# httpsLiem/Spectrogram-YOLOv11

Measured on AMD Instinct MI355X. Metric: spectrogram-images/sec (train fwd+bwd) YOLOv11-s 640², bs=64, 1/2/4/8 GPU, higher is better.
Workload: dtype f16; 1 GPU; configs[2]: YOLOv11-s train fwd+bwd (+clip, SGD-nesterov, EMA) from synthetic IQ through the HIP STFT/log-mel producer; model=yolo11s.yaml, imgsz=640, batch_per_gpu=64, global_batch=64, parallelism=dp1, weights=random-init, nc=80

## Files before the change

### include/sy11.h

```cpp
#ifndef SY11_H
#define SY11_H
#include <stddef.h>
#include <stdint.h>
#ifdef __cplusplus
extern "C" {
#endif

#define SY11_VERSION 100

enum sy11_status { SY11_OK = 0, SY11_EINVAL = -1, SY11_EUNSUPPORTED = -2, SY11_ELAUNCH = -3 };
enum sy11_dtype { SY11_F32 = 0, SY11_F16 = 1, SY11_BF16 = 2, SY11_U8 = 3  };

#define SY11_EPI_SILU 1u
#define SY11_EPI_ACCUM 2u
#define SY11_EPI_OUT_F32 4u

typedef struct sy11_conv_desc {
  int32_t dtype;
  int32_t B, IH, IW, C;
  int32_t x_ld;
  int32_t OH, OW, N;
  int32_t y_ld;
  int32_t KH, KW, SH, SW, PH, PW, DH, DW;
  int32_t groups;
// ... 24 lines not shown
  float* running_var;
  float* mean;
  float* rstd;
  float* scale;
  float* shift;
  int32_t* ticket;
  float eps, momentum;
  double count;
} sy11_bn_tail;
int sy11_conv2d_fwd_bn(const sy11_conv_desc* d, const void* x, const void* w, void* y, float* stat_sum, float* stat_sq,
                       const sy11_bn_tail* bn, void* stream);

int sy11_conv2d_dgrad(const sy11_conv_desc* d, const void* dy, int32_t dy_ld, const void* wt, void* dx, void* stream);

int sy11_conv2d_wgrad(const sy11_conv_desc* d, const void* x, const void* dy, int32_t dy_ld, float* dw, void* stream);

int sy11_weight_transpose(int32_t dtype, int32_t N, int32_t T, int32_t C, const void* w, void* wt, void* stream);

int sy11_weight_transpose_multi(int32_t dtype, int32_t nlayers, int32_t total_tiles, const void* desc, const void* src,
                                void* dst, void* stream);

int sy11_stem_conv_fwd(const sy11_conv_desc* d, const float* x_nchw, const void* w, const float* bias, void* y,
                       float* stat_sum, float* stat_sq, void* stream);
int sy11_stem_conv_fwd_bn(const sy11_conv_desc* d, const float* x_nchw, const void* w, void* y, float* stat_sum,
                          float* stat_sq, const sy11_bn_tail* bn, void* stream);
int sy11_stem_conv_wgrad(const sy11_conv_desc* d, const float* x_nchw, const void* dy, int32_t dy_ld, float* dw,
                         void* stream);


int sy11_bn_finalize(int32_t C, int32_t stat_slots, double count, const float* stat_sum, const float* stat_sq, const float* gamma,
// ... 186 lines not shown
```

### spectrogram-yolov11_amd/csrc/elementwise.hip

```cpp
#include "common.h"
#include "tune.h"
#include "det.h"
#include <type_traits>

template <int I, int N, typename F>
__device__ __forceinline__ void sy11_static_for(F&& f) {
  if constexpr (I < N) {
    f(std::integral_constant<int, I>{});
    sy11_static_for<I + 1, N>(f);
  }
}


template <typename T, int VEC> struct Vec {
  T v[VEC];
};
template <typename T, int VEC>
__device__ __forceinline__ void vload(const T* p, float* f) {
  if constexpr (VEC == 1) {
    f[0] = ElemTraits<T>::to_f(*p);
  } else {
    typedef T vt __attribute__((ext_vector_type(VEC)));
    const vt v = *(const vt*)p;
#pragma unroll
// ... 1134 lines not shown
  float* src = partials;
  int cl = clean ? 1 : 0;
  long sstride = stride;
  float* ping = scratch;
  while (rows > 256) {
    const long nr = (rows + 63) / 64;
    float* dst = ping;
    hipLaunchKernelGGL((fold_stage_kernel<false>), dim3(cdiv(N, 64), (unsigned)nr), dim3(256), 0, st, rows, N, src, sstride, dst, 64L, 0L, 0L, (float*)nullptr, cl);
    src = dst; sstride = N; rows = nr; cl = 0;
    ping = dst + nr * N;
  }
  hipLaunchKernelGGL((fold_stage_kernel<true>), dim3(cdiv(N, 64), 1), dim3(256), 0, st, rows, N, src, sstride, out, rows, 0L, 0L, (float*)nullptr, cl);
  SY11_LAUNCH_CHECK("fold_rows");
  return SY11_OK;
}
```

### spectrogram-yolov11_amd/csrc/wgrad.hip

```cpp
#include "common.h"
#include "tune.h"
#include "det.h"
#include <stdlib.h>

struct WgradArgs {
  const void* x;
  const void* dy;
  float* dw;
  int M, N, K, C, T;
  int x_ld, dy_ld;
  int IH, IW, OH, OW, sy, sx;
  int tiles_k;
  unsigned x_bytes, dy_bytes;
  unsigned mag_ow, mag_oh;
  int tiles, total;
  int pix_per_split;
  long dw_split_stride;
  signed char tap_dy[64];
  signed char tap_dx[64];
};

template <bool STORE>
__device__ __forceinline__ void dw_out(float* p, float v) {
  if (STORE) *p = v; else atomicAdd(p, v);
// ... 640 lines not shown
static int wgrad3x3p_sp(const WgradArgs& a, int ws) { return (ws >= 40 && a.OH % (160 / ws) == 0) ? 160 : 80; }

static int cu_count() {
  static int n = 0;
  if (!n) {
    int dev = 0;
    hipDeviceProp_t p;
    n = (hipGetDevice(&dev) == hipSuccess && hipGetDeviceProperties(&p, dev) == hipSuccess && p.multiProcessorCount > 0) ? p.multiProcessorCount : 256;
  }
  return n;
}

constexpr int WGRAD_NCFG = SY11_WGRAD_NCFG;
static_assert(WGRAD_NCFG == 20, "configuration table and its size (tune.h) out of step");
constexpr int WGRAD_WIDE_LDS = 2 * 64 * ((128 * 2 + 64) + (256 * 2 + 64));
static int wgrad_launch_cfg(WgradArgs a, int dtype, hipStream_t st, int cfg) {
  const int kind = cfg >> 2;
  const bool psplit = kind == 2;
  const bool patch = kind == 3;
  const bool wide = kind == 4;
  if (wide && dtype == SY11_F32) SY11_FAIL(SY11_EUNSUPPORTED, "conv2d_wgrad: configuration %d is 16-bit only", cfg);
  const int patch_ws = patch ? wgrad3x3p_ws(a) : 0;
  if (patch && (!patch_ws || dtype == SY11_F32)) SY11_FAIL(SY11_EUNSUPPORTED, "conv2d_wgrad: configuration %d does not take this shape", cfg);
  const int patch_sp = patch ? wgrad3x3p_sp(a, patch_ws) : 0;
  const int tile = kind == 1 ? 128 : 64;
  const int slots = cu_count() * (wide ? 1 : patch ? (patch_sp == 80 ? 4 : 2) : (tile == 128 ? 2 : 3));
  const int target_wg = (slots << (cfg & 3)) >> 2;
  const int pcb = a.C > 32 ? 64 : 32, pnb = a.N > 32 ? 64 : 32;
  a.tiles_k = patch ? cdiv(a.C, pcb) : cdiv(a.K, wide ? 256 : tile);
  const int tiles = patch ? a.tiles_k * cdiv(a.N, pnb) * 3 : a.tiles_k * cdiv(a.N, wide ? 128 : tile);
  int splits = target_wg / tiles;
  const int stage_px = patch ? patch_sp : 64;
  const int max_splits = cdiv(a.M, 8 * stage_px);
  if (splits > max_splits) splits = max_splits;
  if (splits < 1) splits = 1;
  a.pix_per_split = cdiv(cdiv(a.M, splits), stage_px) * stage_px;
  splits = cdiv(a.M, a.pix_per_split);
  a.tiles = tiles; a.total = tiles * splits;
  DetPartials dp;
  float* const dw_out = a.dw;
  const bool det = sy11_det(8) && splits > 1;
  if (det) {
    if (!dp.acquire(st, 1, splits, a.N * a.K, false)) SY11_FAIL(SY11_ELAUNCH, "conv2d_wgrad: ordered-reduction workspace unavailable (%d x %d floats)", splits, a.N * a.K);
    a.dw = dp.buf(0);
    a.dw_split_stride = (long)a.N * a.K;
  }
  a.mag_ow = (unsigned)(((1u << 20) + a.OW - 1) / a.OW);
  a.mag_oh = (unsigned)(((1u << 20) + a.OH - 1) / a.OH);
  dim3 grid(cdiv(a.total, 8) * 8), block(256);
  if (wide) {
    static bool attr_set = false;
    if (!attr_set) {
      if (hipFuncSetAttribute((const void*)wgrad16w_kernel<_Float16>, hipFuncAttributeMaxDynamicSharedMemorySize, WGRAD_WIDE_LDS) != hipSuccess ||
          hipFuncSetAttribute((const void*)wgrad16w_kernel<__bf16>, hipFuncAttributeMaxDynamicSharedMemorySize, WGRAD_WIDE_LDS) != hipSuccess)
        SY11_FAIL(SY11_ELAUNCH, "conv2d_wgrad: cannot raise the LDS limit to %d bytes", WGRAD_WIDE_LDS);
      attr_set = true;
// ... 21 lines not shown
    } while (0)
    if (dtype == SY11_F16) SY11_WG3(_Float16); else SY11_WG3(__bf16);
#undef SY11_WG3
#undef SY11_WG3B
  } else if (dtype == SY11_F16) {
    if (psplit) hipLaunchKernelGGL((wgrad16_kernel<_Float16, 64, true>), grid, block, 0, st, a);
    else if (tile == 128) hipLaunchKernelGGL((wgrad16_kernel<_Float16, 128>), grid, block, 0, st, a);
    else hipLaunchKernelGGL((wgrad16_kernel<_Float16, 64>), grid, block, 0, st, a);
  } else {
    if (psplit) hipLaunchKernelGGL((wgrad16_kernel<__bf16, 64, true>), grid, block, 0, st, a);
    else if (tile == 128) hipLaunchKernelGGL((wgrad16_kernel<__bf16, 128>), grid, block, 0, st, a);
    else hipLaunchKernelGGL((wgrad16_kernel<__bf16, 64>), grid, block, 0, st, a);
  }
  SY11_LAUNCH_CHECK("conv2d_wgrad");
  if (det) return dp.fold(0, dw_out);
  return SY11_OK;
}

extern "C" int sy11_conv2d_wgrad_dw(const sy11_conv_desc* d, const void* x, const void* dy, int dy_ld, float* dw, hipStream_t st);
extern "C" int sy11_conv2d_wgrad(const sy11_conv_desc* d, const void* x, const void* dy, int32_t dy_ld, float* dw,
                                 void* stream) {
  SY11_REQUIRE(d && x && dy && dw, "conv2d_wgrad: null argument");
  SY11_REQUIRE(dtype_ok(d->dtype), "conv2d_wgrad: bad dtype");
  hipStream_t st = (hipStream_t)stream;
  if (d->groups != 1 && d->groups == d->C && d->C == d->N) return sy11_conv2d_wgrad_dw(d, x, dy, dy_ld, dw, st);
  if (d->groups != 1) {
    SY11_REQUIRE(d->groups > 1 && d->C % d->groups == 0 && d->N % d->groups == 0, "conv2d_wgrad: channels not divisible by groups=%d", d->groups);
    const int cg = d->C / d->groups, ng = d->N / d->groups, es = dtype_size(d->dtype);
    sy11_conv_desc dg = *d;
    dg.groups = 1; dg.C = cg; dg.N = ng;
    for (int g = 0; g < d->groups; ++g) {
      const int rc = sy11_conv2d_wgrad(&dg, (const char*)x + (long)g * cg * es, (const char*)dy + (long)g * ng * es, dy_ld,
                                       dw + (long)g * ng * d->KH * d->KW * cg, stream);
      if (rc) return rc;
    }
    return SY11_OK;
  }
  const int esz = dtype_size(d->dtype), epc = 16 / esz;
  SY11_REQUIRE(d->KH * d->KW <= 64 && d->KH > 0 && d->KW > 0, "conv2d_wgrad: <=64 taps");
  SY11_REQUIRE(d->C % epc == 0 && d->N % epc == 0, "conv2d_wgrad: C and N must be multiples of %d", epc);
  SY11_REQUIRE(d->x_ld % epc == 0 && dy_ld % epc == 0 && d->x_ld >= d->C && dy_ld >= d->N, "conv2d_wgrad: bad pixel strides");
  SY11_REQUIRE((((uintptr_t)x | (uintptr_t)dy) & 15) == 0 && ((uintptr_t)dw & 3) == 0, "conv2d_wgrad: misaligned pointer");
  SY11_REQUIRE((long)d->B * d->IH * d->IW < (1L << 31) && (long)d->B * d->OH * d->OW < (1L << 31), "conv2d_wgrad: pixel count overflows int32");
  WgradArgs a{};
  a.x = x; a.dy = dy; a.dw = dw;
  {
    const long xb = ((long)d->B * d->IH * d->IW - 1) * d->x_ld * esz + (long)d->C * esz;
    const long db = ((long)d->B * d->OH * d->OW - 1) * dy_ld * esz + (long)d->N * esz;
    SY11_REQUIRE(xb < (1L << 31) && db < (1L << 31), "conv2d_wgrad: operand view larger than 2 GiB");
    SY11_REQUIRE((long)(d->OW + 64) * d->OW < (1L << 20) && (long)(d->OH + 64) * d->OH < (1L << 20), "conv2d_wgrad: output map larger than 960 pixels per side");
    a.x_bytes = (unsigned)xb; a.dy_bytes = (unsigned)db;
  }
  a.T = d->KH * d->KW; a.C = d->C; a.K = a.T * a.C; a.N = d->N;
  a.M = d->B * d->OH * d->OW;
  a.x_ld = d->x_ld; a.dy_ld = dy_ld;
  a.IH = d->IH; a.IW = d->IW; a.OH = d->OH; a.OW = d->OW; a.sy = d->SH; a.sx = d->SW;
  for (int r = 0; r < d->KH; ++r)
    for (int s = 0; s < d->KW; ++s) {
      a.tap_dy[r * d->KW + s] = (signed char)(r * d->DH - d->PH);
      a.tap_dx[r * d->KW + s] = (signed char)(s * d->DW - d->PW);
    }
  int cfg = ((a.N > 64 && a.K > 64 && a.M > 30000) ? 4 : 0) + 2;
  if (d->dtype != SY11_F32 && a.M >= 200000 && wgrad3x3p_ws(a)) cfg = 14;
  const int forced = sy11_opt(OPT_WGRAD_CFG);
  const int ncfg = d->dtype == SY11_F32 ? 8 : WGRAD_NCFG;
  auto patch_ok = [&](int c) { return c < 12 || (c < 16 ? wgrad3x3p_ws(a) != 0 : (a.N > 64 && a.K > 128)); };
  if (forced >= 0 && forced < ncfg && patch_ok(forced)) return wgrad_launch_cfg(a, d->dtype, st, forced);
  {
    sy11tune::Cache& cache = sy11tune::cache(1);
    static float* scratch = nullptr;
    static size_t scratch_elems = 0;
    const int key[] = {d->dtype, a.M, a.N, a.K, a.C, a.sy, a.sx, a.IW, a.OW, a.x_ld, a.dy_ld};
    const uint64_t h = sy11tune::hash(key, (int)(sizeof(key) / sizeof(int)));
    int hit;
    if (cache.get(h, &hit)) {
      if (hit >= 0 && hit < ncfg && patch_ok(hit)) cfg = hit;
    } else if (sy11tune::enabled() && !sy11tune::capturing(st)) {
      const size_t need = (size_t)a.N * a.K;
      if (need > scratch_elems) {
        if (scratch) (void)hipFree(scratch);
        scratch = nullptr; scratch_elems = 0;
        if (hipMalloc((void**)&scratch, need * sizeof(float)) == hipSuccess) scratch_elems = need; else (void)hipGetLastError();
      }
      if (scratch) {
        WgradArgs t = a;
        t.dw = scratch;
        int cands[WGRAD_NCFG], nc = 0;
        for (int c = 0; c < ncfg; ++c)
          if (patch_ok(c)) cands[nc++] = c;
        const int best = sy11tune::pick(cands, nc, [&](int c) { return wgrad_launch_cfg(t, d->dtype, st, c); }, st, "wgrad", key,
                                        (int)(sizeof(key) / sizeof(int)));
        if (best >= 0) { cache.put(h, best); cfg = best; }
      }
    }
  }
  return wgrad_launch_cfg(a, d->dtype, st, cfg);
}
```

### spectrogram-yolov11_amd/sy11/_lib.py

```python
from __future__ import annotations

import ctypes as C
import os
from pathlib import Path

_HERE = Path(__file__).resolve().parent
LIB_PATH = Path(os.environ.get("SY11_LIB", _HERE / "libsy11.so"))

F32, F16, BF16, U8 = 0, 1, 2, 3
EPI_SILU, EPI_ACCUM, EPI_OUT_F32 = 1, 2, 4


class Sy11Error(RuntimeError):
    pass


class ConvDesc(C.Structure):
    _fields_ = [(n, C.c_int32) for n in (
        "dtype", "B", "IH", "IW", "C", "x_ld", "OH", "OW", "N", "y_ld",
        "KH", "KW", "SH", "SW", "PH", "PW", "DH", "DW", "groups")] + [("flags", C.c_uint32), ("stat_slots", C.c_int32)]


class BnTail(C.Structure):
    _fields_ = [(n, C.c_void_p) for n in ("gamma", "beta", "running_mean", "running_var", "mean", "rstd", "scale", "shift", "ticket")] \
# ... 20 lines not shown
    _fields_ = [("m0", C.c_int64), ("out_off", C.c_int64), ("M", C.c_int32), ("log2d", C.c_int32), ("dphi", C.c_uint32),
                ("reserved", C.c_int32)]


_vp, _i32, _i64, _f32, _f64, _u32 = C.c_void_p, C.c_int32, C.c_int64, C.c_float, C.c_double, C.c_uint32
_dp = C.POINTER(ConvDesc)
_bp = C.POINTER(BnTail)
_op = C.POINTER(OptDesc)

SIGNATURES = {
    "sy11_conv2d_fwd": [_dp, _vp, _vp, _vp, _vp, _vp, _vp, _vp],
    "sy11_conv2d_fwd_bn": [_dp, _vp, _vp, _vp, _vp, _vp, _bp, _vp],
    "sy11_stem_conv_fwd_bn": [_dp, _vp, _vp, _vp, _vp, _vp, _bp, _vp],
    "sy11_conv2d_dgrad": [_dp, _vp, _i32, _vp, _vp, _vp],
    "sy11_conv2d_wgrad": [_dp, _vp, _vp, _i32, _vp, _vp],
    "sy11_weight_transpose": [_i32, _i32, _i32, _i32, _vp, _vp, _vp],
    "sy11_weight_transpose_multi": [_i32, _i32, _i32, _vp, _vp, _vp, _vp],
    "sy11_stem_conv_fwd": [_dp, _vp, _vp, _vp, _vp, _vp, _vp, _vp],
    "sy11_stem_conv_wgrad": [_dp, _vp, _vp, _i32, _vp, _vp],
    "sy11_bn_finalize": [_i32, _i32, _f64, _vp, _vp, _vp, _vp, _f32, _f32, _vp, _vp, _vp, _vp, _vp, _vp, _vp],
    "sy11_bn_act_fwd": [_i32, _i64, _i32, _vp, _i32, _vp, _vp, _i32, _vp, _i32, _vp, _i32, _vp],
    "sy11_bn_act_bwd_reduce": [_i32, _i64, _i32, _vp, _i32, _vp, _i32, _vp, _vp, _vp, _vp, _i32, _vp, _vp, _i32, _vp],
    "sy11_bn_act_bwd_apply": [_i32, _i64, _i32, _vp, _i32, _vp, _i32, _vp, _vp, _vp, _vp, _vp, _i32, _vp, _vp, _i32,
                              _vp, _i32, _vp, _vp, _vp],
    "sy11_bn_act_bwd_apply_res": [_i32, _i64, _i32, _vp, _i32, _vp, _i32, _vp, _vp, _vp, _vp, _vp, _i32, _vp, _vp, _i32,
                                  _vp, _i32, _vp, _vp, _vp, _i32, _i32, _vp],
    "sy11_copy2d": [_i32, _i64, _i32, _vp, _i32, _vp, _i32, _i32, _vp],
    "sy11_upsample2x_fwd": [_i32, _i32, _i32, _i32, _i32, _vp, _i32, _vp, _i32, _vp],
    "sy11_upsample2x_bwd": [_i32, _i32, _i32, _i32, _i32, _vp, _i32, _vp, _i32, _i32, _vp],
    "sy11_box_iou": [_i32, _i32, _vp, _vp, _f32, _vp, _vp],
# ... 44 lines not shown
    "sy11_tune_import": [_vp, _i64],
    "sy11_tune_clear": [],
    "sy11_peak_mfma_f16": [_i32, _i32, _vp, _vp],
    "sy11_debug_stamps": [_vp],
    "sy11_debug_stamps_persistent": [_vp],
    "sy11_opt_workspace_floats": [_i32],
    "sy11_opt_grad_norm": [_i64, _vp, _vp, _vp, _vp, _i32, _vp],
    "sy11_opt_step": [_op, _vp, _vp, _vp, _vp, _vp, _vp, _vp, _vp, _vp, _vp, _vp, _vp, _vp],
})
OTHER = {"sy11_version": ([], C.c_int), "sy11_last_error": ([], C.c_char_p),
         "sy11_nms_workspace_bytes": ([_i32], C.c_size_t),
         "sy11_nms_batched_workspace_bytes": ([_i32, _vp], C.c_size_t),
         "sy11_scan_merge_workspace_bytes": ([_i32, _i32], C.c_size_t),
         "sy11_attention_workspace_bytes": ([_i32, _i32, _i32], C.c_size_t),
         "sy11_iq_extract_tile": ([_i32], C.c_int32),
         "sy11_tune_export": ([_vp, _i64], C.c_int64)}

_lib = None


def load():
    global _lib
    if _lib is not None:
        return _lib
    if not LIB_PATH.exists():
        raise Sy11Error(f"libsy11.so not found at {LIB_PATH}: build it with "
                        f"`make -C spectrogram-yolov11_amd/csrc` (or __graft_entry__.build()). "
                        f"There is no CPU / PyTorch fallback for the hot path.")
    import torch
    lib = C.CDLL(str(LIB_PATH))
    for name, args in SIGNATURES.items():
# ... 63 lines not shown
```

### spectrogram-yolov11_amd/sy11/engine/__init__.py

```python
from __future__ import annotations

import os

from typing import List, Optional

import torch

from .. import ops


class Act:

    __slots__ = ("_data", "root", "c0", "_grad", "_ready", "raw", "req", "_dtype")

    def __init__(self, data: Optional[torch.Tensor], root: Optional["Act"] = None, c0: int = 0,
                 raw: Optional[torch.Tensor] = None, req: bool = True, dtype=None):
        self._data = data
        self.root = root
        self.c0 = c0
        self._grad = None
        self._ready = False
        self.raw = raw
        self.req = req
        self._dtype = dtype
# ... 45 lines not shown
        r = self._root_grad()
        if not r._ready:
            r._grad.zero_()
            r._ready = True
        return r._grad if self.root is None else r._grad[..., self.c0:self.c0 + self.C]

    def set_grad(self, g: torch.Tensor):
        assert self.root is None
        self._grad = g
        self._ready = True


_SIDE_WGRAD = os.environ.get("SY11_WGRAD_STREAM", "32") != "0"
_SIDE_BATCH = max(int(os.environ.get("SY11_WGRAD_STREAM", "32") or 0), 1)
_SIDE_STREAMS = {}


def _side_stream(device):
    d = torch.device(device)
    key = d.index if d.index is not None else torch.cuda.current_device()
    if key not in _SIDE_STREAMS:
        _SIDE_STREAMS[key] = torch.cuda.Stream(device=d)
    return _SIDE_STREAMS[key]


_BRANCH_STREAMS_ON = os.environ.get("SY11_BRANCH_STREAMS", "0") != "0"
_BRANCH_STREAMS = {}


def _branch_stream(device, b):
# ... 45 lines not shown
        self.pool_off = 0
        self.pool_need = 0
        self.bn_counters: List[torch.Tensor] = []
        self.capturing = False
        self.w_views = None
        self.wt_views = None
        self.w_bank = None
        self.flat_state = None
        self.side = None
        self.side_refs: List = []
        self.use_side = _SIDE_WGRAD and device is not None and torch.device(device).type == "cuda"
        self.use_branches = _BRANCH_STREAMS_ON and device is not None and torch.device(device).type == "cuda"
        self.open_branches = set()
        self.main_stream = None
        self.tape_branches: List = []

    def on_side(self, fn, *keep):
        if not self.use_side:
            fn()
            return
        if self.side is None:
            self.side = _side_stream(self.device)
            self.side_queue = []
        self.side_queue.append(fn)
        self.side_refs.append(keep)
        if len(self.side_queue) >= _SIDE_BATCH:
            self.flush_side()

    def flush_side(self):
        if self.side is None or not self.side_queue:
# ... 106 lines not shown
                v = seg.view(p.shape)
            self.views[id(p)] = v
            self.offsets[id(p)] = off
            off += pad(n)

    def begin_backward(self, device):
        if self.flat is None or self.flat.device != device:
            self._build(device)
        fresh = any(p.grad is None or p.grad.data_ptr() != self.views[id(p)].data_ptr() for p in self.params)
        if fresh:
            if not (self.external_zero and all(p.grad is not None for p in self.params)):
                self.flat.zero_()
            for p in self.params:
                p.grad = self.views[id(p)]

    def grad_krsc(self, p: torch.nn.Parameter) -> torch.Tensor:
        return self.views[id(p)].permute(0, 2, 3, 1)

    def grad_vec(self, p: torch.nn.Parameter) -> torch.Tensor:
        return self.views[id(p)]


def engine_dtype(module) -> torch.dtype:
    if torch.is_autocast_enabled("cuda"):
        return torch.get_autocast_dtype("cuda")
    return getattr(module, "_sy11_dtype", torch.float32)


def to_act(t: torch.Tensor, dtype) -> Act:
    if not t.is_cuda:
# ... 36 lines not shown
        out = module._run(ec, acts if is_list else acts[0])
        if ec.bn_counters:
            torch._foreach_add_(ec.bn_counters, 1)
        ctx.module = module
        outs, out_list = _flatten(out)
        ctx.ec, ctx.acts, ctx.outs, ctx.n_in = ec, acts, outs, n_in
        ctx.n_t = len(tensors)
        ctx.in_req = [t.requires_grad for t in ins]
        return tuple(from_act(a) for a in outs)

    @staticmethod
    def backward(ctx, *gouts):
        ec: Ctx = ctx.ec
        if ec.grads is not None:
            ec.grads.begin_backward(ec.device)
        for a, g in zip(ctx.outs, gouts):
            if g is None or a.data.dim() != 4:
                continue
            gv = g.permute(0, 2, 3, 1)
            if gv.dtype != a.data.dtype or not gv.is_contiguous():
                gv = gv.to(a.data.dtype).contiguous()
            a.set_grad(gv)
        hook = module_post_backward.get(id(ec.grads)) if ec.grads is not None else None
        mark = ec.marks.get("bucket") if (hook is not None and getattr(hook, "staged", False)) else None
        def first_bucket():
            ec.join_side()
            hook(ec.grads, 0)
        ec.run_tape(len(ec.tape) - 1, 0, mark, first_bucket if mark is not None else None)
        ec.join_side()
        ec.tape.clear()
        ctx.module.__dict__["_sy11_pool_hint"] = ec.pool_need
        gin = []
        for a, req in zip(ctx.acts, ctx.in_req):
            if req:
                g = a.grad_read().permute(0, 3, 1, 2)
                gin.append(g.float() if g.dtype != torch.float32 else g)
            else:
                gin.append(None)
        if hook is not None:
            hook(ec.grads, 1)
        return (None, None, None, None, None, *gin, *([None] * (ctx.n_t - ctx.n_in)))


module_post_backward = {}
# ... 22 lines not shown
                ec = Ctx(True, True, dtype, dev, store, module.__dict__.get("_sy11_pool_hint", 0))
                ec.capturing = True
                ec.attach_flat(module)
                acts = [to_act(t, dtype) for t in self.static_in]
                out = module._run(ec, acts if is_list else acts[0])
                if ec.bn_counters:
                    torch._foreach_add_(ec.bn_counters, 1)
            self.ec, self.acts = ec, acts
            self.outs, _ = _flatten(out)
            self.static_out = [from_act(a) for a in self.outs]
            self.static_gout = [torch.zeros_like(a.data) for a in self.outs]
            hook = module_post_backward.get(id(store))
            mark = ec.marks.get("bucket") if (hook is not None and getattr(hook, "staged", False)) else None
            if mark is not None and not (0 < mark < len(ec.tape)):
                mark = None
            self.g_bwd = torch.cuda.CUDAGraph()
            self.g_bwd2 = None
            with torch.cuda.graph(self.g_bwd, pool=self.g_fwd.pool(), stream=side, capture_error_mode=_CAPTURE_MODE):
                for a, g in zip(self.outs, self.static_gout):
                    if a.data.dim() == 4:
                        a.set_grad(g)
                ec.run_tape(len(ec.tape) - 1, mark if mark is not None else 0)
                ec.join_side()
                if mark is None:
                    self.static_gin = [a.grad_read().permute(0, 3, 1, 2) if a.req else None for a in acts]
            if mark is not None:
                self.g_bwd2 = torch.cuda.CUDAGraph()
                with torch.cuda.graph(self.g_bwd2, pool=self.g_fwd.pool(), stream=side, capture_error_mode=_CAPTURE_MODE):
                    ec.run_tape(mark - 1, 0)
                    ec.join_side()
                    self.static_gin = [a.grad_read().permute(0, 3, 1, 2) if a.req else None for a in acts]
            ec.tape.clear()
        torch.cuda.current_stream(dev).wait_stream(side)


class _GraphedFwd:

    def __init__(self, module, xs, is_list, dtype):
        dev = xs[0].device
        self.static_in = [x.detach().clone() for x in xs]
        side = torch.cuda.Stream(device=dev)
        side.wait_stream(torch.cuda.current_stream(dev))
        with torch.cuda.stream(side):
            self.g_fwd = torch.cuda.CUDAGraph()
            with torch.cuda.graph(self.g_fwd, stream=side, capture_error_mode=_CAPTURE_MODE):
# ... 113 lines not shown
```

### spectrogram-yolov11_amd/sy11/nn/modules/conv.py

```python
from __future__ import annotations

import math

import torch
import torch.nn as nn

from ... import ops
from ...engine import Act, Ctx, run_module

import os

_BN_TAIL = os.environ.get("SY11_BN_TAIL", "0") != "0"
_BN_STAT_SLOTS = max(1, int(os.environ.get("SY11_BN_STAT_SLOTS", "32")))

__all__ = ("Conv", "DWConv", "DDWConv", "Concat", "WeightedSpatialAttention", "GCT", "Fusion", "autopad")


def autopad(k, p=None, d=1):
    if d > 1:
        k = d * (k - 1) + 1 if isinstance(k, int) else [d * (x - 1) + 1 for x in k]
    if p is None:
        p = k // 2 if isinstance(k, int) else [x // 2 for x in k]
    return p

# ... 156 lines not shown
            tail = (B * OH * OW, gamma, beta, bn.eps, mom, rm, rv, mean, rstd, scale, shift, ec.zeros(max(g, 1)))
            if stem:
                ops.stem_conv_fwd_bn(x.raw, w, y, s, p, (st[0], st[1]), tail)
            else:
                ops.conv2d_fwd_bn(x.data, w, y, k, s, p, d, g, (st[0], st[1]), tail)
        else:
            if stem:
                ops.stem_conv_fwd(x.raw, w, y, s, p, stats=(st[0], st[1]))
            else:
                ops.conv2d_fwd(x.data, w, y, k, s, p, d, g, stats=(st[0], st[1]))
            ops.bn_finalize(B * OH * OW, st[0], st[1], gamma, beta, bn.eps, mom, rm, rv, mean, rstd, scale, shift)
        if track and bn.num_batches_tracked is not None:
            ec.bn_counters.append(bn.num_batches_tracked)
        ops.bn_act_fwd(y, scale, shift, out.data, silu=silu, res=res.data if res is not None else None)
        if ec.record:
            def bw():
                gs = ec.grads
                dz = out.grad_read()
                sg = ec.zeros(2, 8 if B * OH * OW >= 8192 else 1, N)
                ops.bn_act_bwd_reduce(y, dz, mean, rstd, scale, shift, silu, sg[0], sg[1])
                dy = torch.empty_like(y)
                has_bn = id(bn.weight) in gs.views
                rg, acc = res.grad_for_write() if (res is not None and res.req) else (None, False)
                ops.bn_act_bwd_apply(y, dz, mean, rstd, scale, shift, gamma, silu, sg[0], sg[1], dy,
                                     gs.grad_vec(bn.weight) if has_bn else None, gs.grad_vec(bn.bias) if has_bn else None,
                                     res_grad=rg, res_accumulate=acc)
                if id(conv.weight) in gs.views:
                    dw = gs.grad_krsc(conv.weight)
                    if stem:
                        ec.on_side(lambda: ops.stem_conv_wgrad(x.raw, dy, dw, s, p), x.raw, dy)
                    elif padded:
                        dwp = torch.zeros(tuple(w.shape), dtype=torch.float32, device=ec.device)
                        ops.conv2d_wgrad(x.data, dy, dwp, k, s, p, d, g)
                        dw.add_(dwp[..., :C1])
                    else:
                        xd = x.data
                        ec.on_side(lambda: ops.conv2d_wgrad(xd, dy, dw, k, s, p, d, g), xd, dy)
                if padded and x_real.req:
                    gp = torch.zeros_like(x.data)
                    ops.conv2d_dgrad(dy, ops.weight_transpose(w), gp, (B, OH, OW, N), k, s, p, d, 1, accumulate=True)
                    gx, acc = x_real.grad_for_write()
                    if acc:
                        gx.add_(gp[..., :C1])
                    else:
                        gx.copy_(gp[..., :C1])
                if x.req:
                    gx, acc = x.grad_for_write()
                    if g == 1 or g != C1 or g != N:
                        if ops.dgrad_leaves_holes(k, s, p, d) and not acc:
                            gx.zero_()
                            acc = True
                        wtr = ec.transposed(conv.weight, w) if g == 1 else ops.weight_transpose(w, g)
# ... 147 lines not shown
```

### spectrogram-yolov11_amd/sy11/ops.py

```python
from __future__ import annotations

import ctypes as C

import numpy as np
import torch

from . import _lib
from ._lib import EPI_ACCUM, EPI_OUT_F32, EPI_SILU, BnTail, ConvDesc, OptDesc, call

_DT = {torch.float32: _lib.F32, torch.float16: _lib.F16, torch.bfloat16: _lib.BF16}


def dt_code(t: torch.dtype) -> int:
    try:
        return _DT[t]
    except KeyError:
        raise _lib.Sy11Error(f"unsupported dtype {t}") from None


def _stream():
    return C.c_void_p(torch.cuda.current_stream().cuda_stream)


def _p(t):
# ... 98 lines not shown

def conv2d_dgrad(dy, w_or_wt, dx, y_shape, k, s=1, p=0, d=1, groups=1, accumulate=False):
    _need_gpu(dy, w_or_wt, dx)
    dsc = _desc(dx.shape, view_ld(dx), y_shape, y_shape[-1], dy.dtype, k, s, p, d, groups, EPI_ACCUM if accumulate else 0)
    call("sy11_conv2d_dgrad", C.byref(dsc), _p(dy), view_ld(dy), _p(w_or_wt), _p(dx), _stream())
    return dx


def conv2d_wgrad(x, dy, dw_f32, k, s=1, p=0, d=1, groups=1):
    _need_gpu(x, dy, dw_f32)
    if dw_f32.dtype != torch.float32 or not dw_f32.is_contiguous():
        raise _lib.Sy11Error("conv2d_wgrad: dw must be a contiguous f32 tensor")
    dsc = _desc(x.shape, view_ld(x), dy.shape, view_ld(dy), x.dtype, k, s, p, d, groups, 0)
    call("sy11_conv2d_wgrad", C.byref(dsc), _p(x), _p(dy), view_ld(dy), _p(dw_f32), _stream())
    return dw_f32


def stem_conv_fwd(x_nchw, w_krsc, y, s=2, p=1, bias=None, stats=None, silu=False):
    _need_gpu(x_nchw, w_krsc, y)
    if x_nchw.dtype != torch.float32 or not x_nchw.is_contiguous() or x_nchw.shape[1] != 3:
        raise _lib.Sy11Error("stem_conv_fwd: x must be a contiguous NCHW f32 image with 3 channels")
    B, _, IH, IW = x_nchw.shape
    slots = stats[0].shape[0] if (stats and stats[0].dim() == 2) else 1
    dsc = _desc((B, IH, IW, 3), 3, y.shape, view_ld(y), y.dtype, 3, s, p, 1, 1, EPI_SILU if silu else 0, slots)
    call("sy11_stem_conv_fwd", C.byref(dsc), _p(x_nchw), _p(w_krsc), _p(bias), _p(y), _p(stats[0]) if stats else None,
         _p(stats[1]) if stats else None, _stream())
    return y


def stem_conv_wgrad(x_nchw, dy, dw_f32, s=2, p=1):
# ... 702 lines not shown
```

Before: 3061 spectrogram-images/s.

## Store split-K wgrad partials in an arena and fold all layers in one kernel

Split-K weight-gradient kernels used to accumulate into the f32 gradient buffer with atomicAdd from every split. Now each eligible non-grouped conv writes its per-split partials with plain stores into a per-layer block of a shared arena. After backward, one batched grad_fold kernel sums the splits into the flat gradient buffer. This replaces atomic contention with plain stores and one vectorised reduction pass. The cost is extra arena memory (up to 64 MB per layer), extra read traffic for the fold, and a tuning key that now depends on whether partials are used.

```diff
diff --git a/include/sy11.h b/include/sy11.h
--- a/include/sy11.h
+++ b/include/sy11.h
@@ -62,6 +62,12 @@
 int sy11_conv2d_dgrad(const sy11_conv_desc* d, const void* dy, int32_t dy_ld, const void* wt, void* dx, void* stream);
 
 int sy11_conv2d_wgrad(const sy11_conv_desc* d, const void* x, const void* dy, int32_t dy_ld, float* dw, void* stream);
+
+int sy11_conv2d_wgrad_split(const sy11_conv_desc* d, const void* x, const void* dy, int32_t dy_ld, float* dw, float* partial,
+                            int64_t partial_floats, int32_t* splits_out, void* stream);
+int64_t sy11_conv2d_wgrad_partial_floats(const sy11_conv_desc* d);
+int sy11_grad_fold(const int64_t* table, const int32_t* work, int32_t work_count, const uint16_t* counts, int32_t n_counts,
+                   int32_t entry_base, float* flat, const float* arena, void* stream);
 
 int sy11_weight_transpose(int32_t dtype, int32_t N, int32_t T, int32_t C, const void* w, void* wt, void* stream);
 
diff --git a/spectrogram-yolov11_amd/csrc/elementwise.hip b/spectrogram-yolov11_amd/csrc/elementwise.hip
--- a/spectrogram-yolov11_amd/csrc/elementwise.hip
+++ b/spectrogram-yolov11_amd/csrc/elementwise.hip
@@ -1172,3 +1172,61 @@
   SY11_LAUNCH_CHECK("fold_rows");
   return SY11_OK;
 }
+
+struct GradFoldCounts { uint16_t c[256]; };
+__global__ __launch_bounds__(256) void grad_fold_kernel(const int64_t* __restrict__ table, const int32_t* __restrict__ work, const GradFoldCounts cnt,
+                                                        int entry_base, float* __restrict__ flat, const float* __restrict__ arena) {
+  const int e = work[2 * blockIdx.x], chunk = work[2 * blockIdx.x + 1];
+  const int S = cnt.c[e - entry_base];
+  if (S == 0) return;
+  const int64_t* ent = table + 3L * e;
+  const long i = ((long)chunk * 256 + threadIdx.x) * 4;
+  if (i >= ent[2]) return;
+  const long nk = ent[2];
+  const float* __restrict__ src = arena + ent[1] + i;
+  float* dst = flat + ent[0] + i;
+  f32x4 t[4];
+#pragma unroll
+  for (int q = 0; q < 4; ++q) t[q] = f32x4{0.f, 0.f, 0.f, 0.f};
+  int s = 0;
+  for (; s + 8 <= S; s += 8) {
+    f32x4 v[8];
+#pragma unroll
+    for (int j = 0; j < 8; ++j) v[j] = *(const f32x4*)(src + (long)(s + j) * nk);
+#pragma unroll
+    for (int j = 0; j < 8; ++j) t[j & 3] += v[j];
+  }
+  for (; s + 4 <= S; s += 4) {
+    f32x4 v[4];
+#pragma unroll
+    for (int j = 0; j < 4; ++j) v[j] = *(const f32x4*)(src + (long)(s + j) * nk);
+#pragma unroll
+    for (int j = 0; j < 4; ++j) t[j] += v[j];
+  }
+#pragma unroll
+  for (int j = 0; j < 3; ++j)
+    if (s + j < S) t[j] += *(const f32x4*)(src + (long)(s + j) * nk);
+  const f32x4 tot = ((t[0] + t[1]) + t[2]) + t[3];
+  f32x4 d = *(const f32x4*)dst;
+  d += tot;
+  *(f32x4*)dst = d;
+}
+
+extern "C" int sy11_grad_fold(const int64_t* table, const int32_t* work, int32_t work_count, const uint16_t* counts, int32_t n_counts,
+                              int32_t entry_base, float* flat, const float* arena, void* stream) {
+  SY11_REQUIRE(work_count >= 0 && n_counts >= 0 && n_counts <= 256 && entry_base >= 0, "grad_fold: at most 256 entries per launch (got %d)", n_counts);
+  if (work_count == 0 || n_counts == 0) return SY11_OK;
+  SY11_REQUIRE(table && work && counts && flat && arena, "grad_fold: null argument");
+  SY11_REQUIRE((((uintptr_t)flat | (uintptr_t)arena) & 15) == 0, "grad_fold: flat buffer and arena must be 16-byte aligned");
+  GradFoldCounts c{};
+  bool any = false;
+  for (int i = 0; i < n_counts; ++i) {
+    SY11_REQUIRE(counts[i] <= 256, "grad_fold: split count %d of entry %d exceeds 256", (int)counts[i], entry_base + i);
+    c.c[i] = counts[i];
+    any = any || counts[i] != 0;
+  }
+  if (!any) return SY11_OK;
+  hipLaunchKernelGGL(grad_fold_kernel, dim3((unsigned)work_count), dim3(256), 0, (hipStream_t)stream, table, work, c, (int)entry_base, flat, arena);
+  SY11_LAUNCH_CHECK("grad_fold");
+  return SY11_OK;
+}
diff --git a/spectrogram-yolov11_amd/csrc/wgrad.hip b/spectrogram-yolov11_amd/csrc/wgrad.hip
--- a/spectrogram-yolov11_amd/csrc/wgrad.hip
+++ b/spectrogram-yolov11_amd/csrc/wgrad.hip
@@ -678,14 +678,13 @@
 constexpr int WGRAD_NCFG = SY11_WGRAD_NCFG;
 static_assert(WGRAD_NCFG == 20, "configuration table and its size (tune.h) out of step");
 constexpr int WGRAD_WIDE_LDS = 2 * 64 * ((128 * 2 + 64) + (256 * 2 + 64));
-static int wgrad_launch_cfg(WgradArgs a, int dtype, hipStream_t st, int cfg) {
+static int wgrad_geometry(WgradArgs& a, int dtype, int cfg, int* patch_ws_out = nullptr, int* patch_sp_out = nullptr) {
   const int kind = cfg >> 2;
-  const bool psplit = kind == 2;
   const bool patch = kind == 3;
   const bool wide = kind == 4;
-  if (wide && dtype == SY11_F32) SY11_FAIL(SY11_EUNSUPPORTED, "conv2d_wgrad: configuration %d is 16-bit only", cfg);
+  if ((wide || patch) && dtype == SY11_F32) return 0;
   const int patch_ws = patch ? wgrad3x3p_ws(a) : 0;
-  if (patch && (!patch_ws || dtype == SY11_F32)) SY11_FAIL(SY11_EUNSUPPORTED, "conv2d_wgrad: configuration %d does not take this shape", cfg);
+  if (patch && !patch_ws) return 0;
   const int patch_sp = patch ? wgrad3x3p_sp(a, patch_ws) : 0;
   const int tile = kind == 1 ? 128 : 64;
   const int slots = cu_count() * (wide ? 1 : patch ? (patch_sp == 80 ? 4 : 2) : (tile == 128 ? 2 : 3));
@@ -701,9 +700,32 @@
   a.pix_per_split = cdiv(cdiv(a.M, splits), stage_px) * stage_px;
   splits = cdiv(a.M, a.pix_per_split);
   a.tiles = tiles; a.total = tiles * splits;
+  if (patch_ws_out) *patch_ws_out = patch_ws;
+  if (patch_sp_out) *patch_sp_out = patch_sp;
+  return splits;
+}
+
+static int wgrad_launch_cfg(WgradArgs a, int dtype, hipStream_t st, int cfg, float* partial = nullptr, size_t partial_floats = 0,
+                            int* splits_out = nullptr) {
+  if (splits_out) *splits_out = 0;
+  const int kind = cfg >> 2;
+  const bool psplit = kind == 2;
+  const bool patch = kind == 3;
+  const bool wide = kind == 4;
+  if (wide && dtype == SY11_F32) SY11_FAIL(SY11_EUNSUPPORTED, "conv2d_wgrad: configuration %d is 16-bit only", cfg);
+  if (patch && (!wgrad3x3p_ws(a) || dtype == SY11_F32)) SY11_FAIL(SY11_EUNSUPPORTED, "conv2d_wgrad: configuration %d does not take this shape", cfg);
+  int patch_ws = 0, patch_sp = 0;
+  const int tile = kind == 1 ? 128 : 64;
+  const int pcb = a.C > 32 ? 64 : 32, pnb = a.N > 32 ? 64 : 32;
+  const int splits = wgrad_geometry(a, dtype, cfg, &patch_ws, &patch_sp);
   DetPartials dp;
   float* const dw_out = a.dw;
   const bool det = sy11_det(8) && splits > 1;
+  const bool store = partial && sy11_opt(OPT_DETERMINISTIC) == 0 && splits >= 2 && splits <= 256 && (size_t)splits * a.N * a.K <= partial_floats;
+  if (store) {
+    a.dw = partial;
+    a.dw_split_stride = (long)a.N * a.K;
+  }
   if (det) {
     if (!dp.acquire(st, 1, splits, a.N * a.K, false)) SY11_FAIL(SY11_ELAUNCH, "conv2d_wgrad: ordered-reduction workspace unavailable (%d x %d floats)", splits, a.N * a.K);
     a.dw = dp.buf(0);
@@ -755,12 +777,27 @@
   }
   SY11_LAUNCH_CHECK("conv2d_wgrad");
   if (det) return dp.fold(0, dw_out);
+  if (store && splits_out) *splits_out = splits;
   return SY11_OK;
 }
 
 extern "C" int sy11_conv2d_wgrad_dw(const sy11_conv_desc* d, const void* x, const void* dy, int dy_ld, float* dw, hipStream_t st);
-extern "C" int sy11_conv2d_wgrad(const sy11_conv_desc* d, const void* x, const void* dy, int32_t dy_ld, float* dw,
-                                 void* stream) {
+
+static void wgrad_problem(const sy11_conv_desc* d, WgradArgs& a) {
+  a.T = d->KH * d->KW; a.C = d->C; a.K = a.T * a.C; a.N = d->N;
+  a.M = d->B * d->OH * d->OW;
+  a.IH = d->IH; a.IW = d->IW; a.OH = d->OH; a.OW = d->OW; a.sy = d->SH; a.sx = d->SW;
+  for (int r = 0; r < d->KH; ++r)
+    for (int s = 0; s < d->KW; ++s) {
+      a.tap_dy[r * d->KW + s] = (signed char)(r * d->DH - d->PH);
+      a.tap_dx[r * d->KW + s] = (signed char)(s * d->DW - d->PW);
+    }
+}
+static bool wgrad_cfg_takes(const WgradArgs& a, int c) { return c < 12 || (c < 16 ? wgrad3x3p_ws(a) != 0 : (a.N > 64 && a.K > 128)); }
+
+static int wgrad_entry(const sy11_conv_desc* d, const void* x, const void* dy, int32_t dy_ld, float* dw, float* partial, size_t partial_floats,
+                       int* splits_out, void* stream) {
+  if (splits_out) *splits_out = 0;
   SY11_REQUIRE(d && x && dy && dw, "conv2d_wgrad: null argument");
   SY11_REQUIRE(dtype_ok(d->dtype), "conv2d_wgrad: bad dtype");
   hipStream_t st = (hipStream_t)stream;
@@ -783,6 +820,8 @@
   SY11_REQUIRE(d->x_ld % epc == 0 && dy_ld % epc == 0 && d->x_ld >= d->C && dy_ld >= d->N, "conv2d_wgrad: bad pixel strides");
   SY11_REQUIRE((((uintptr_t)x | (uintptr_t)dy) & 15) == 0 && ((uintptr_t)dw & 3) == 0, "conv2d_wgrad: misaligned pointer");
   SY11_REQUIRE((long)d->B * d->IH * d->IW < (1L << 31) && (long)d->B * d->OH * d->OW < (1L << 31), "conv2d_wgrad: pixel count overflows int32");
+  if (partial && (sy11_opt(OPT_DETERMINISTIC) != 0 || partial_floats == 0)) partial = nullptr;
+  SY11_REQUIRE(!partial || ((uintptr_t)partial & 15) == 0, "conv2d_wgrad_split: the partial block must be 16-byte aligned");
   WgradArgs a{};
   a.x = x; a.dy = dy; a.dw = dw;
   {
@@ -792,27 +831,21 @@
     SY11_REQUIRE((long)(d->OW + 64) * d->OW < (1L << 20) && (long)(d->OH + 64) * d->OH < (1L << 20), "conv2d_wgrad: output map larger than 960 pixels per side");
     a.x_bytes = (unsigned)xb; a.dy_bytes = (unsigned)db;
   }
-  a.T = d->KH * d->KW; a.C = d->C; a.K = a.T * a.C; a.N = d->N;
-  a.M = d->B * d->OH * d->OW;
+  wgrad_problem(d, a);
   a.x_ld = d->x_ld; a.dy_ld = dy_ld;
-  a.IH = d->IH; a.IW = d->IW; a.OH = d->OH; a.OW = d->OW; a.sy = d->SH; a.sx = d->SW;
-  for (int r = 0; r < d->KH; ++r)
-    for (int s = 0; s < d->KW; ++s) {
-      a.tap_dy[r * d->KW + s] = (signed char)(r * d->DH - d->PH);
-      a.tap_dx[r * d->KW + s] = (signed char)(s * d->DW - d->PW);
-    }
   int cfg = ((a.N > 64 && a.K > 64 && a.M > 30000) ? 4 : 0) + 2;
   if (d->dtype != SY11_F32 && a.M >= 200000 && wgrad3x3p_ws(a)) cfg = 14;
   const int forced = sy11_opt(OPT_WGRAD_CFG);
   const int ncfg = d->dtype == SY11_F32 ? 8 : WGRAD_NCFG;
-  auto patch_ok = [&](int c) { return c < 12 || (c < 16 ? wgrad3x3p_ws(a) != 0 : (a.N > 64 && a.K > 128)); };
-  if (forced >= 0 && forced < ncfg && patch_ok(forced)) return wgrad_launch_cfg(a, d->dtype, st, forced);
+  auto patch_ok = [&](int c) { return wgrad_cfg_takes(a, c); };
+  if (forced >= 0 && forced < ncfg && patch_ok(forced)) return wgrad_launch_cfg(a, d->dtype, st, forced, partial, partial_floats, splits_out);
   {
     sy11tune::Cache& cache = sy11tune::cache(1);
     static float* scratch = nullptr;
     static size_t scratch_elems = 0;
-    const int key[] = {d->dtype, a.M, a.N, a.K, a.C, a.sy, a.sx, a.IW, a.OW, a.x_ld, a.dy_ld};
-    const uint64_t h = sy11tune::hash(key, (int)(sizeof(key) / sizeof(int)));
+    const int key[] = {d->dtype, a.M, a.N, a.K, a.C, a.sy, a.sx, a.IW, a.OW, a.x_ld, a.dy_ld, 1};
+    const int nkey = (int)(sizeof(key) / sizeof(int)) - (partial ? 0 : 1);
+    const uint64_t h = sy11tune::hash(key, nkey);
     int hit;
     if (cache.get(h, &hit)) {
       if (hit >= 0 && hit < ncfg && patch_ok(hit)) cfg = hit;
@@ -829,11 +862,46 @@
         int cands[WGRAD_NCFG], nc = 0;
         for (int c = 0; c < ncfg; ++c)
           if (patch_ok(c)) cands[nc++] = c;
-        const int best = sy11tune::pick(cands, nc, [&](int c) { return wgrad_launch_cfg(t, d->dtype, st, c); }, st, "wgrad", key,
-                                        (int)(sizeof(key) / sizeof(int)));
+        const int best = sy11tune::pick(cands, nc, [&](int c) {
+          int sp = 0;
+          const int rc = wgrad_launch_cfg(t, d->dtype, st, c, partial, partial_floats, &sp);
+          if (rc || sp == 0) return rc;
+          return sy11_fold_rows_ordered(sp, (int)need, partial, (long)need, scratch, nullptr, st);
+        }, st, "wgrad", key, nkey);
         if (best >= 0) { cache.put(h, best); cfg = best; }
       }
     }
   }
-  return wgrad_launch_cfg(a, d->dtype, st, cfg);
-}
+  return wgrad_launch_cfg(a, d->dtype, st, cfg, partial, partial_floats, splits_out);
+}
+
+extern "C" int sy11_conv2d_wgrad(const sy11_conv_desc* d, const void* x, const void* dy, int32_t dy_ld, float* dw,
+                                 void* stream) {
+  return wgrad_entry(d, x, dy, dy_ld, dw, nullptr, 0, nullptr, stream);
+}
+
+extern "C" int sy11_conv2d_wgrad_split(const sy11_conv_desc* d, const void* x, const void* dy, int32_t dy_ld, float* dw, float* partial,
+                                       int64_t partial_floats, int32_t* splits_out, void* stream) {
+  SY11_REQUIRE(splits_out, "conv2d_wgrad_split: null splits_out");
+  SY11_REQUIRE(partial_floats >= 0 && (partial || partial_floats == 0), "conv2d_wgrad_split: bad partial block");
+  int sp = 0;
+  const int rc = wgrad_entry(d, x, dy, dy_ld, dw, partial, (size_t)partial_floats, &sp, stream);
+  *splits_out = sp;
+  return rc;
+}
+
+extern "C" int64_t sy11_conv2d_wgrad_partial_floats(const sy11_conv_desc* d) {
+  if (!d || !dtype_ok(d->dtype) || d->groups != 1 || d->KH <= 0 || d->KW <= 0 || d->KH * d->KW > 64) return 0;
+  WgradArgs a{};
+  wgrad_problem(d, a);
+  if (a.M <= 0 || a.N <= 0 || a.K <= 0) return 0;
+  const int ncfg = d->dtype == SY11_F32 ? 8 : WGRAD_NCFG;
+  int64_t best = 0;
+  for (int c = 0; c < ncfg; ++c) {
+    if (!wgrad_cfg_takes(a, c)) continue;
+    WgradArgs t = a;
+    const int splits = wgrad_geometry(t, d->dtype, c);
+    if (splits >= 2 && splits <= 256) { const int64_t f = (int64_t)splits * a.N * a.K; if (f > best) best = f; }
+  }
+  return best;
+}
diff --git a/spectrogram-yolov11_amd/sy11/_lib.py b/spectrogram-yolov11_amd/sy11/_lib.py
--- a/spectrogram-yolov11_amd/sy11/_lib.py
+++ b/spectrogram-yolov11_amd/sy11/_lib.py
@@ -58,6 +58,8 @@
     "sy11_stem_conv_fwd_bn": [_dp, _vp, _vp, _vp, _vp, _vp, _bp, _vp],
     "sy11_conv2d_dgrad": [_dp, _vp, _i32, _vp, _vp, _vp],
     "sy11_conv2d_wgrad": [_dp, _vp, _vp, _i32, _vp, _vp],
+    "sy11_conv2d_wgrad_split": [_dp, _vp, _vp, _i32, _vp, _vp, _i64, C.POINTER(C.c_int32), _vp],
+    "sy11_grad_fold": [_vp, _vp, _i32, C.POINTER(C.c_uint16), _i32, _i32, _vp, _vp, _vp],
     "sy11_weight_transpose": [_i32, _i32, _i32, _i32, _vp, _vp, _vp],
     "sy11_weight_transpose_multi": [_i32, _i32, _i32, _vp, _vp, _vp, _vp],
     "sy11_stem_conv_fwd": [_dp, _vp, _vp, _vp, _vp, _vp, _vp, _vp],
@@ -132,7 +134,8 @@
          "sy11_scan_merge_workspace_bytes": ([_i32, _i32], C.c_size_t),
          "sy11_attention_workspace_bytes": ([_i32, _i32, _i32], C.c_size_t),
          "sy11_iq_extract_tile": ([_i32], C.c_int32),
-         "sy11_tune_export": ([_vp, _i64], C.c_int64)}
+         "sy11_tune_export": ([_vp, _i64], C.c_int64),
+         "sy11_conv2d_wgrad_partial_floats": ([_dp], C.c_int64)}
 
 _lib = None
 
diff --git a/spectrogram-yolov11_amd/sy11/engine/__init__.py b/spectrogram-yolov11_amd/sy11/engine/__init__.py
--- a/spectrogram-yolov11_amd/sy11/engine/__init__.py
+++ b/spectrogram-yolov11_amd/sy11/engine/__init__.py
@@ -2,6 +2,7 @@
 
 import os
 
+from types import SimpleNamespace
 from typing import List, Optional
 
 import torch
@@ -83,6 +84,8 @@
 _SIDE_WGRAD = os.environ.get("SY11_WGRAD_STREAM", "32") != "0"
 _SIDE_BATCH = max(int(os.environ.get("SY11_WGRAD_STREAM", "32") or 0), 1)
 _SIDE_STREAMS = {}
+_WGRAD_PARTIALS = os.environ.get("SY11_WGRAD_PARTIALS", "1") != "0"
+_WGRAD_BLOCK_CAP = (64 << 20) // 4
 
 
 def _side_stream(device):
@@ -158,6 +161,15 @@
         self.open_branches = set()
         self.main_stream = None
         self.tape_branches: List = []
+        self.wg_layers: List = []
+        self.wg_seen = set()
+        self.wg_plan = None
+        self.wg_counts: List = []
+
+    def wgrad_register(self, w, x_shape, y_shape, k, s, p, d):
+        if _WGRAD_PARTIALS and self.grads is not None and id(w) not in self.wg_seen:
+            self.wg_seen.add(id(w))
+            self.wg_layers.append((w, ops.wgrad_partial_floats(x_shape, y_shape, self.dtype, k, s, p, d)))
 
     def on_side(self, fn, *keep):
         if not self.use_side:
@@ -294,6 +306,49 @@
             for p in self.params:
                 p.grad = self.views[id(p)]
 
+    def wgrad_begin(self, ec):
+        ec.wg_plan, ec.wg_counts = None, []
+        if not ec.wg_layers or self.flat is None or ops._lib.get_option("deterministic"):
+            return
+        key = tuple((id(w), cap) for w, cap in ec.wg_layers)
+        plans = self.__dict__.setdefault("_wg_plans", {})
+        plan = plans.get(key)
+        if plan is None:
+            entries, blocks, index, off = [], [], {}, 0
+            for w, cap in ec.wg_layers:
+                n = min(cap, _WGRAD_BLOCK_CAP) // 4 * 4
+                if id(w) not in self.offsets or n < 2 * w.numel() or w.numel() % 4 or self.offsets[id(w)] % 4:
+                    continue
+                index[id(w)] = len(entries)
+                entries.append((self.offsets[id(w)], off, w.numel()))
+                blocks.append((off, n))
+                off += n
+            arena = self.__dict__.get("_wg_arena")
+            if entries and (arena is None or arena.numel() < off or arena.device != self.flat.device):
+                arena = torch.empty(off, dtype=torch.float32, device=self.flat.device)
+                self.__dict__["_wg_arena"] = arena
+            table, work, first = ops.grad_fold_tables(entries, self.flat.device) if entries else (None, None, [0])
+            plan = SimpleNamespace(index=index, blocks=blocks, arena=arena if entries else None, table=table, work=work, first=first,
+                                   floats=off)
+            plans[key] = plan
+        ec.wg_plan = plan
+        ec.wg_counts = [0] * len(plan.blocks)
+
+    def wgrad(self, ec, w, x, dy, dw, k, s, p, d):
+        plan = ec.wg_plan
+        e = plan.index.get(id(w)) if plan is not None else None
+        if e is None or ec.wg_counts[e]:
+            ops.conv2d_wgrad(x, dy, dw, k, s, p, d, 1)
+            return
+        off, n = plan.blocks[e]
+        ec.wg_counts[e] = ops.conv2d_wgrad_split(x, dy, dw, plan.arena[off:off + n], k, s, p, d, 1)
+
+    def wgrad_fold(self, ec):
+        plan = ec.wg_plan
+        if plan is not None and any(ec.wg_counts):
+            ops.grad_fold(plan.table, plan.work, plan.first, ec.wg_counts, self.flat, plan.arena)
+            ec.wg_counts = [0] * len(ec.wg_counts)
+
     def grad_krsc(self, p: torch.nn.Parameter) -> torch.Tensor:
         return self.views[id(p)].permute(0, 2, 3, 1)
 
@@ -360,6 +415,7 @@
         ec: Ctx = ctx.ec
         if ec.grads is not None:
             ec.grads.begin_backward(ec.device)
+            ec.grads.wgrad_begin(ec)
         for a, g in zip(ctx.outs, gouts):
             if g is None or a.data.dim() != 4:
                 continue
@@ -371,9 +427,12 @@
         mark = ec.marks.get("bucket") if (hook is not None and getattr(hook, "staged", False)) else None
         def first_bucket():
             ec.join_side()
+            ec.grads.wgrad_fold(ec)
             hook(ec.grads, 0)
         ec.run_tape(len(ec.tape) - 1, 0, mark, first_bucket if mark is not None else None)
         ec.join_side()
+        if ec.grads is not None:
+            ec.grads.wgrad_fold(ec)
         ec.tape.clear()
         ctx.module.__dict__["_sy11_pool_hint"] = ec.pool_need
         gin = []
@@ -426,6 +485,7 @@
             mark = ec.marks.get("bucket") if (hook is not None and getattr(hook, "staged", False)) else None
             if mark is not None and not (0 < mark < len(ec.tape)):
                 mark = None
+            store.wgrad_begin(ec)
             self.g_bwd = torch.cuda.CUDAGraph()
             self.g_bwd2 = None
             with torch.cuda.graph(self.g_bwd, pool=self.g_fwd.pool(), stream=side, capture_error_mode=_CAPTURE_MODE):
@@ -434,6 +494,7 @@
                         a.set_grad(g)
                 ec.run_tape(len(ec.tape) - 1, mark if mark is not None else 0)
                 ec.join_side()
+                store.wgrad_fold(ec)
                 if mark is None:
                     self.static_gin = [a.grad_read().permute(0, 3, 1, 2) if a.req else None for a in acts]
             if mark is not None:
@@ -441,6 +502,7 @@
                 with torch.cuda.graph(self.g_bwd2, pool=self.g_fwd.pool(), stream=side, capture_error_mode=_CAPTURE_MODE):
                     ec.run_tape(mark - 1, 0)
                     ec.join_side()
+                    store.wgrad_fold(ec)
                     self.static_gin = [a.grad_read().permute(0, 3, 1, 2) if a.req else None for a in acts]
             ec.tape.clear()
         torch.cuda.current_stream(dev).wait_stream(side)
diff --git a/spectrogram-yolov11_amd/sy11/nn/modules/conv.py b/spectrogram-yolov11_amd/sy11/nn/modules/conv.py
--- a/spectrogram-yolov11_amd/sy11/nn/modules/conv.py
+++ b/spectrogram-yolov11_amd/sy11/nn/modules/conv.py
@@ -194,6 +194,8 @@
             ec.bn_counters.append(bn.num_batches_tracked)
         ops.bn_act_fwd(y, scale, shift, out.data, silu=silu, res=res.data if res is not None else None)
         if ec.record:
+            if g == 1 and not stem and not padded:
+                ec.wgrad_register(conv.weight, (B, H, W, C1), (B, OH, OW, N), k, s, p, d)
             def bw():
                 gs = ec.grads
                 dz = out.grad_read()
@@ -215,7 +217,10 @@
                         dw.add_(dwp[..., :C1])
                     else:
                         xd = x.data
-                        ec.on_side(lambda: ops.conv2d_wgrad(xd, dy, dw, k, s, p, d, g), xd, dy)
+                        if g == 1:
+                            ec.on_side(lambda: gs.wgrad(ec, conv.weight, xd, dy, dw, k, s, p, d), xd, dy)
+                        else:
+                            ec.on_side(lambda: ops.conv2d_wgrad(xd, dy, dw, k, s, p, d, g), xd, dy)
                 if padded and x_real.req:
                     gp = torch.zeros_like(x.data)
                     ops.conv2d_dgrad(dy, ops.weight_transpose(w), gp, (B, OH, OW, N), k, s, p, d, 1, accumulate=True)
diff --git a/spectrogram-yolov11_amd/sy11/ops.py b/spectrogram-yolov11_amd/sy11/ops.py
--- a/spectrogram-yolov11_amd/sy11/ops.py
+++ b/spectrogram-yolov11_amd/sy11/ops.py
@@ -136,6 +136,54 @@
     dsc = _desc(x.shape, view_ld(x), dy.shape, view_ld(dy), x.dtype, k, s, p, d, groups, 0)
     call("sy11_conv2d_wgrad", C.byref(dsc), _p(x), _p(dy), view_ld(dy), _p(dw_f32), _stream())
     return dw_f32
+
+
+def conv2d_wgrad_split(x, dy, dw_f32, partial, k, s=1, p=0, d=1, groups=1) -> int:
+    _need_gpu(x, dy, dw_f32, partial)
+    if dw_f32.dtype != torch.float32 or not dw_f32.is_contiguous():
+        raise _lib.Sy11Error("conv2d_wgrad_split: dw must be a contiguous f32 tensor")
+    if partial.dtype != torch.float32 or not partial.is_contiguous():
+        raise _lib.Sy11Error("conv2d_wgrad_split: the partial block must be a contiguous f32 tensor")
+    dsc = _desc(x.shape, view_ld(x), dy.shape, view_ld(dy), x.dtype, k, s, p, d, groups, 0)
+    n = C.c_int32(0)
+    call("sy11_conv2d_wgrad_split", C.byref(dsc), _p(x), _p(dy), view_ld(dy), _p(dw_f32), _p(partial), partial.numel(), C.byref(n), _stream())
+    return int(n.value)
+
+
+def wgrad_partial_floats(x_shape, y_shape, dtype, k, s=1, p=0, d=1, groups=1) -> int:
+    B, IH, IW, Cn = x_shape
+    _, OH, OW, N = y_shape
+    dsc = ConvDesc(dt_code(dtype), B, IH, IW, Cn, Cn, OH, OW, N, N, k, k, s, s, p, p, d, d, groups, 0, 1)
+    return int(_lib.load().sy11_conv2d_wgrad_partial_floats(C.byref(dsc)))
+
+
+FOLD_CHUNK = 1024
+FOLD_ENTRIES = 256
+
+
+def grad_fold_tables(entries, device):
+    tab = np.asarray(entries, dtype=np.int64).reshape(-1, 3)
+    if tab.size and (tab % 4).any():
+        raise _lib.Sy11Error("grad_fold: offsets and sizes must be multiples of 4 floats")
+    work, first = [], []
+    for e, (_, _, nk) in enumerate(tab.tolist()):
+        first.append(len(work))
+        work.extend((e, c) for c in range(-(-nk // FOLD_CHUNK)))
+    first.append(len(work))
+    wk = np.asarray(work, dtype=np.int32).reshape(-1, 2)
+    return torch.from_numpy(tab).to(device), torch.from_numpy(wk).to(device), first
+
+
+def grad_fold(table, work, first, counts, flat, arena, lo=0, hi=None):
+    _need_gpu(table, work, flat, arena)
+    hi = len(counts) if hi is None else hi
+    for e0 in range(lo, hi, FOLD_ENTRIES):
+        e1 = min(e0 + FOLD_ENTRIES, hi)
+        if not any(counts[e0:e1]):
+            continue
+        cs = (C.c_uint16 * (e1 - e0))(*counts[e0:e1])
+        w0, w1 = first[e0], first[e1]
+        call("sy11_grad_fold", _p(table), C.c_void_p(work.data_ptr() + 8 * w0), w1 - w0, cs, e1 - e0, e0, _p(flat), _p(arena), _stream())
 
 
 def stem_conv_fwd(x_nchw, w_krsc, y, s=2, p=1, bias=None, stats=None, silu=False):
```

Result: no change. 3052 spectrogram-images/s (-0.3%).
